# duyhominhnguyen/conan-fgw

Hardware: AMD Instinct MI355X
Metric: molecules/s (K=5 conformers) (higher is better)
Workload: dtype f32

## Files before the change

### conan-fgw_amd/csrc/fgw.hip

```cpp
#include "fgw_coupling.h"
#ifdef CONAN_FGW_PROFILE
FGW_PROF_ACCESSOR(conan_debug_fgw_prof_large)
FGW_PROF_TRACE_ACCESSOR(conan_debug_fgw_trace_large)
#endif

namespace {

__global__ void k_fgw_init(const float *__restrict__ Cs, const float *__restrict__ init_C, const float *__restrict__ init_Y,
                           FgwDims D, int max_iter, double *__restrict__ Cw, double *__restrict__ Yw, int *__restrict__ active,
                           int *__restrict__ info, float *__restrict__ errs, float *__restrict__ Yout, float *__restrict__ Cout, FgwAdj adj) {
    const int b = blockIdx.x;
    const int NN = D.N * D.N, Nd = D.N * D.d;
    if (!init_C && adj.rowptr) {
        const int N = D.N, g = b * D.K;
        for (int t = threadIdx.x; t < NN; t += blockDim.x) Cout[(size_t)b * NN + t] = 0.f;
        __syncthreads();
        const int lo = adj.gptr[g], n = min(adj.gptr[g + 1] - lo, N);
        for (int e = adj.rowptr[lo] + (int)threadIdx.x; e < adj.rowptr[lo + n]; e += blockDim.x) {
            const int i = adj.tgt[e] - lo, j = adj.col[e] - lo;
            if (i >= 0 && i < N && j >= 0 && j < N) atomicAdd(&Cout[(size_t)b * NN + j * N + i], 1.0f);
        }
        __threadfence_block();
        __syncthreads();
        for (int t = threadIdx.x; t < NN; t += blockDim.x) Cw[(size_t)b * NN + t] = (double)Cout[(size_t)b * NN + t];
// ... 587 lines not shown
    w.redo = region(BK * 4 + 512);
    w.dense = region(ragged ? al256(BK * NN * sizeof(float)) : 0);
    w.asym = region(solver == 2 && symmetric != 1 ? al256(conan_fgw_bapg_asym_scratch_bytes(B, K, N)) : 0);
    w.total = end;
    return w;
}

enum class FgwPath {
    Small,
    Big,
    General,
    Bapg
};
struct FgwPlan {
    FgwPath path;
    int mode;
    size_t lds_bytes;
    bool kl, ppa, asym;
    bool y_from_t;
    size_t big_bytes;
    bool big_u8, big_wpc2, big_ordered;
};

template <int M>
void launch_general(const FgwCall &c, const FgwPlan &pl, int outer, int y_zero, const int *only) {
    auto go = [&](auto kernel, int blocks) {
        launch_lds(kernel, blocks, 64 * GEN_NW, pl.lds_bytes, c.s, c.Ys, c.Cs, c.ps, c.p, c.D, c.prm, outer, y_zero | (c.symmetric < 0 ? 2 : 0), c.Cw,
                   c.Yw, c.active, c.T, c.info, c.scratch, c.Ypart, c.Cpart, only, c.adj);
    };
    if (only) go(k_fgw_coupling<M, false, GEN_NW, true>, (c.D.B * c.D.K + 63) / 64);
    else with_flags([&](auto KL, auto PPA, auto ASYM) { go(k_fgw_coupling<M, KL.value, GEN_NW, false, PPA.value, ASYM.value>, c.D.B * c.D.K); },
                    pl.kl, pl.ppa, pl.asym);
}

int fgw_fwd_impl(const float *Ys, const float *Cs, const float *ps, const float *p, const float *lambdas, const float *init_C,
                 const float *init_Y, int B, int K, int N, int d, const conan_fgw_params *params, float *Y, float *C, float *T, float *T_iter,
                 int *info, float *errs, void *workspace, void *stream, FgwAdj adj, int solver, int symmetric) {
    if (solver < 0 || solver > 2 || symmetric < -1 || symmetric > 1) return CONAN_E_BADARG;
    if (!Ys || !(Cs || (adj.gptr && adj.rowptr && adj.col && adj.tgt)) || !params || !Y || !C || !T || !info || !errs || !workspace || B <= 0 || K <= 0 || N <= 0 || d <= 0)
        return CONAN_E_BADARG;
    if (params->max_iter <= 0 || params->num_iter_max <= 0) return CONAN_E_BADARG;
    if (params->fixed_features && !init_Y) return CONAN_E_BADARG;
    if (params->loss_fun != 0 && params->loss_fun != 1) return CONAN_E_BADARG;
    const bool ragged = adj.rowptr != nullptr, small = conan_fgw_small_supported(N, d), kl = params->loss_fun != 0;
    const bool model = solver == 0 && symmetric == 1;
    const FgwWorkspace w = fgw_workspace(B, K, N, d, ragged, solver, symmetric);
    const size_t NN = (size_t)N * N, NP = (size_t)N * pitch_of(N);
    FgwCall c{};
    c.Ys = Ys; c.Cs = Cs; c.ps = ps; c.p = p; c.lambdas = lambdas; c.init_C = init_C; c.init_Y = init_Y;
    c.D = FgwDims{B, K, N, d, pitch_of(N)};
    c.prm = *params;
    c.adj = adj;
    c.symmetric = symmetric;
    c.Y = Y; c.C = C; c.T = T; c.info = info; c.errs = errs;
    c.Cw = ws_at<double>(workspace, w.Cw); c.Yw = ws_at<double>(workspace, w.Yw); c.active = ws_at<int>(workspace, w.active);
    c.scratch = ws_at<char>(workspace, w.scratch); c.scratch_stride = coupling_scratch_stride(NP);
    c.Ypart = ws_at<fgw_part_t>(workspace, w.Ypart); c.Cpart = ws_at<fgw_part_t>(workspace, w.Cpart);
    c.redo = ws_at<int>(workspace, w.redo);
    c.asym_scratch = ws_at<char>(workspace, w.asym);
    c.s = as_stream(stream);
    if (ragged) {
        c.prm.cs_small_int = 1;
        c.adj.dense = ws_at<float>(workspace, w.dense);
        if (!(model && !kl && (small ? conan_fgw_fast_supported(N, d, 1) : big_lds(N, true) <= LDS_LIMIT))) {
            k_adj_dense<<<B * K, 256, 0, c.s>>>(c.adj, N);
            c.Cs = c.adj.dense;
            c.adj.rowptr = nullptr;
        }
    }
    if (!model) c.adj = FgwAdj{};
    if (c.adj.rowptr && !kl && (B & 7) == 0 && B <= 4096 && (small || (CONAN_FGW_BIG_ORDER && big_lds(N, true) <= LDS_LIMIT)))
        c.adj.order = ws_at<int>(workspace, w.order);

    FgwPlan pl{};
    pl.kl = kl; pl.ppa = solver == 1; pl.asym = symmetric != 1;
    pl.big_u8 = c.prm.cs_small_int != 0;
    pl.big_bytes = big_lds(N, pl.big_u8);
    pl.path = solver == 2 ? FgwPath::Bapg : model && small ? FgwPath::Small : model && !kl && pl.big_bytes <= LDS_LIMIT ? FgwPath::Big : FgwPath::General;
    pl.mode = general_mode(N, &pl.lds_bytes);
    pl.big_wpc2 = BIG_WPC2 && (B * K <= CONAN_FGW_WPC2_MAX || (CONAN_FGW_WPC2_ORDERED && c.adj.order));
    pl.big_ordered = c.adj.order != nullptr && (B * K & 7) == 0 && pl.big_wpc2 && pl.big_u8;
    pl.y_from_t = pl.path == FgwPath::Small && !c.prm.fixed_features && conan_fgw_update_chunk(K, N, d, B) > 0;
    if (pl.path == FgwPath::Small) { c.zvec = ws_at<double>(workspace, w.zvec); c.yvec = ws_at<double>(workspace, w.yvec); }

    if (pl.path == FgwPath::Small) conan_fgw_small_prepare(c);
    else k_fgw_init<<<B, 256, 0, c.s>>>(c.Cs, init_C, init_Y, c.D, c.prm.max_iter, c.Cw, c.Yw, c.active, info, errs, Y, C, c.adj);
    const FastConst fc = fast_const(c.prm, N);
    for (int outer = 0; outer < c.prm.max_iter; ++outer) {
        const int y_zero = (outer == 0 && !init_Y) ? 1 : 0;
        const int *only = nullptr;
        if (pl.path == FgwPath::Big) {
            auto big = [&](auto kernel) {
                launch_lds(kernel, B * K, 64 * GEN_NW, pl.big_bytes, c.s, c.Ys, c.Cs, c.ps, c.p, c.D, c.prm, fc, outer, y_zero, c.Cw, c.Yw, c.active, c.T,
                           c.info, c.scratch, c.Ypart, c.Cpart, c.redo, c.adj);
            };
            if (pl.big_ordered) big(k_fgw_coupling_big<GEN_NW, true, 2, true>);
            else if (pl.big_u8) { if (pl.big_wpc2) big(k_fgw_coupling_big<GEN_NW, true, 2, false>); else big(k_fgw_coupling_big<GEN_NW, true, 3, false>); }
            else { if (pl.big_wpc2) big(k_fgw_coupling_big<GEN_NW, false, 2, false>); else big(k_fgw_coupling_big<GEN_NW, false, 3, false>); }
            only = c.redo;
        }
        if (pl.path == FgwPath::Small) conan_fgw_small_coupling(c, outer, y_zero, pl.y_from_t ? nullptr : c.Ypart);
        else if (pl.path == FgwPath::Bapg) conan_fgw_bapg_coupling(c, outer, y_zero);
        else if (pl.mode == 2) launch_general<2>(c, pl, outer, y_zero, only);
        else if (pl.mode == 1) launch_general<1>(c, pl, outer, y_zero, only);
        else launch_general<0>(c, pl, outer, y_zero, only);
        if (T_iter)
            (void)hipMemcpyAsync(T_iter + (size_t)outer * B * K * NN, T, (size_t)B * K * NN * sizeof(float), hipMemcpyDeviceToDevice, c.s);
        conan_fgw_small_update(c, outer, pl.y_from_t);
    }
    CONAN_LAUNCH_CHECK();
    return CONAN_OK;
}

}

extern "C" {

long long conan_fgw_workspace_bytes(int B, int K, int N, int d, int ragged, int solver, int symmetric) {
    if (ragged != 0 && ragged != 1) return 0;
    return (long long)fgw_workspace(B, K, N, d, ragged != 0, solver, symmetric).total;
}

int conan_fgw_barycenter_fwd(const float *Ys, const float *Cs, const float *ps, const float *p, const float *lambdas,
                             const float *init_C, const float *init_Y, int B, int K, int N, int d,
                             const conan_fgw_params *params, int solver, int symmetric, float *Y, float *C, float *T, float *T_iter,
                             int *info, float *errs, void *workspace, void *stream) {
    return fgw_fwd_impl(Ys, Cs, ps, p, lambdas, init_C, init_Y, B, K, N, d, params, Y, C, T, T_iter, info, errs, workspace, stream, FgwAdj{}, solver,
                        symmetric);
}

int conan_fgw_barycenter_fwd_ragged(const float *Ys, const int *graph_ptr, const int *rowptr, const int *col, const int *tgt, const float *ps,
                                    const float *p, const float *lambdas, const float *init_C, const float *init_Y, int B, int K, int N, int d,
                                    const conan_fgw_params *params, int solver, int symmetric, float *Y, float *C, float *T, float *T_iter,
                                    int *info, float *errs, void *workspace, void *stream) {
    return fgw_fwd_impl(Ys, nullptr, ps, p, lambdas, init_C, init_Y, B, K, N, d, params, Y, C, T, T_iter, info, errs, workspace, stream,
                        FgwAdj{graph_ptr, rowptr, col, tgt, nullptr, nullptr}, solver, symmetric);
}

int conan_fgw_barycenter_bwd(const float *T, const float *dY, const float *p, const float *lambdas, int B, int K,
                             int N, int d, float *dYs, void *stream) {
    if (!T || !dY || !dYs || B <= 0 || K <= 0 || N <= 0 || d <= 0) return CONAN_E_BADARG;
    const size_t bw_lds = ((size_t)N * N + (size_t)N * d) * sizeof(float);
    if (bw_lds <= 64 * 1024) k_fgw_bwd<true><<<B * K, 256, bw_lds, as_stream(stream)>>>(T, dY, p, lambdas, K, N, d, dYs);
    else k_fgw_bwd<false><<<B * K, 256, 0, as_stream(stream)>>>(T, dY, p, lambdas, K, N, d, dYs);
    CONAN_LAUNCH_CHECK();
    return CONAN_OK;
}

int conan_fgw_densify(const float *feat, const int *graph_ptr, const int *rowptr, const int *col, int num_graphs,
                      int N, int d, float shift, float a, float b, float *Ys, float *Cs, float *minmax, void *stream) {
    if (!feat || !graph_ptr || !Ys || !minmax || num_graphs <= 0 || N <= 0 || d <= 0 || (Cs && (!rowptr || !col))) return CONAN_E_BADARG;
    k_densify<<<num_graphs, 256, 0, as_stream(stream)>>>(feat, graph_ptr, rowptr, col, N, d, shift, a, b, Ys, Cs, minmax);
    CONAN_LAUNCH_CHECK();
    return CONAN_OK;
}

int conan_fgw_densify_bwd(const float *feat, const float *dYs, const int *graph_ptr, const float *minmax,
                          int num_graphs, int N, int d, float shift, float a, float b, float *dfeat, void *stream) {
    if (!feat || !dYs || !graph_ptr || !minmax || !dfeat || num_graphs <= 0 || N <= 0 || d <= 0) return CONAN_E_BADARG;
    k_densify_bwd<<<num_graphs, 256, 0, as_stream(stream)>>>(feat, dYs, graph_ptr, minmax, N, d, shift, a, b, dfeat);
    CONAN_LAUNCH_CHECK();
    return CONAN_OK;
}

int conan_fgw_readout_fwd(const float *Y, int B, int K, int N, int d, int mode, float *out, void *stream) {
    if (!Y || !out || B <= 0 || K <= 0 || N <= 0 || d <= 0 || mode < 0 || mode > 1) return CONAN_E_BADARG;
// ... 15 lines not shown
```

### conan-fgw_amd/csrc/fgw_common.h

```cpp
#pragma once
#include <type_traits>
#include "common.h"

#ifdef CONAN_FGW_PROFILE
static __device__ long long g_fgw_prof[32];
#define FGW_PROF_ACCESSOR(name)                                                          \
    extern "C" int name(long long *out, int reset) {                                     \
        if (out && hipMemcpyFromSymbol(out, HIP_SYMBOL(g_fgw_prof), sizeof(long long) * 32) != hipSuccess) return -2; \
        if (reset) { long long z[32] = {0}; if (hipMemcpyToSymbol(HIP_SYMBOL(g_fgw_prof), z, sizeof(z)) != hipSuccess) return -2; } \
        return 0;                                                                        \
    }
static __device__ long long g_fgw_trace[2 + 6 * 8192];
#define FGW_PROF_TRACE_ACCESSOR(name)                                                    \
    extern "C" int name(long long *out, int reset) {                                     \
        if (out && hipMemcpyFromSymbol(out, HIP_SYMBOL(g_fgw_trace), sizeof(long long) * (2 + 6 * 8192)) != hipSuccess) return -2; \
        if (reset) { long long z[2] = {0, 0}; if (hipMemcpyToSymbol(HIP_SYMBOL(g_fgw_trace), z, sizeof(z)) != hipSuccess) return -2; } \
        return 0;                                                                        \
    }
#define FGW_PROF_TRACE(tag)                                                              \
    do {                                                                                 \
        if (threadIdx.x == 0) {                                                          \
            const unsigned long long i_ = atomicAdd(reinterpret_cast<unsigned long long *>(&g_fgw_trace[0]), 1ull); \
            if (i_ < 8192) {                                                             \
                long long *r_ = &g_fgw_trace[2 + 6 * i_];                                \
                r_[0] = (long long)blockIdx.x; r_[1] = (long long)(tag);                 \
                r_[2] = (long long)__builtin_amdgcn_s_getreg(4 | (31 << 11));            \
                r_[3] = (long long)__builtin_amdgcn_s_getreg(20 | (31 << 11));           \
                r_[4] = prof_w0; r_[5] = wall_clock64();                                 \
            }                                                                            \
        }                                                                                \
    } while (0)
#define FGW_PROF_DECL long long prof_t = wall_clock64(); const long long prof_w0 = prof_t, prof_c0 = clock64(); long long prof_acc[11] = {0, 0, 0, 0, 0, 0, 0, 0, 0, 0, 0}
#define FGW_PROF(k)                                                                      \
    do {                                                                                 \
        const long long t_ = wall_clock64();                                             \
        prof_acc[k] += t_ - prof_t;                                                      \
        prof_t = t_;                                                                     \
    } while (0)
#define FGW_PROF_FLUSH                                                                   \
    do {                                                                                 \
        if (threadIdx.x == 0) {                                                          \
            for (int k_ = 0; k_ < 11; ++k_) atomicAdd(reinterpret_cast<unsigned long long *>(&g_fgw_prof[k_]), (unsigned long long)prof_acc[k_]); \
            atomicAdd(reinterpret_cast<unsigned long long *>(&g_fgw_prof[20]), (unsigned long long)(clock64() - prof_c0));      \
            atomicAdd(reinterpret_cast<unsigned long long *>(&g_fgw_prof[21]), (unsigned long long)(wall_clock64() - prof_w0)); \
        }                                                                                \
    } while (0)
#elif defined(CONAN_FGW_MARK)
#define FGW_PROF_DECL
#define FGW_PROF(k) asm volatile("; FGWMARK " #k)
#define FGW_PROF_FLUSH
#define FGW_PROF_TRACE(tag)
#else
#define FGW_PROF_DECL
#define FGW_PROF(k)
#define FGW_PROF_FLUSH
#define FGW_PROF_TRACE(tag)
#endif

constexpr int FGW_THREADS = 256;
constexpr int FGW_WAVES = FGW_THREADS / 64;

typedef double fgw_part_t;

__host__ __device__ inline int fgw_pitch(int N) { return N | 1; }
struct FgwDims {
    int B, K, N, d, P;
};

struct FgwPair {
    const float *M;
    float *errs;
    int nerr;
};

__device__ __forceinline__ bool fgw_active(const int *__restrict__ active, int B, int b, int outer) {
    const int *a = active + ((outer + 1) & 1) * 2 * B;
    return (a[b] | a[B + b]) != 0;
}
__device__ __forceinline__ void fgw_active_init(int *__restrict__ active, int B, int b) { active[2 * B + b] = 1; active[3 * B + b] = 1; }

struct FgwAdj {
    const int *gptr, *rowptr, *col, *tgt;
    float *dense;
    int *order;
};
template <int NT>
__device__ __forceinline__ void adj_scatter_lds_bytes(const FgwAdj &A, int g, int N, int P, unsigned char *m, int tid) {
    const int lo = A.gptr[g], n = min(A.gptr[g + 1] - lo, N);
    const int e0 = A.rowptr[lo], e1 = A.rowptr[lo + n];
    for (int e = e0 + tid; e < e1; e += NT) {
        const int i = A.tgt[e] - lo, j = A.col[e] - lo;
        if (i >= 0 && i < N && j >= 0 && j < N) {
            const unsigned o = (unsigned)(j * P + i);
            atomicAdd(reinterpret_cast<unsigned *>(m + (o & ~3u)), 1u << (8 * (o & 3u)));
        }
    }
}
template <int NT>
__device__ __forceinline__ const float *adj_dense_slice(const FgwAdj &A, int g, int N, int tid) {
    float *dst = A.dense + (size_t)g * N * N;
    for (int t = tid; t < N * N; t += NT) dst[t] = 0.f;
    __syncthreads();
    const int lo = A.gptr[g], n = min(A.gptr[g + 1] - lo, N);
    const int e0 = A.rowptr[lo], e1 = A.rowptr[lo + n];
    for (int e = e0 + tid; e < e1; e += NT) {
        const int i = A.tgt[e] - lo, j = A.col[e] - lo;
        if (i >= 0 && i < N && j >= 0 && j < N) atomicAdd(&dst[j * N + i], 1.0f);
    }
    __threadfence_block();
    __syncthreads();
    return dst;
}

struct FastConst {
    double two_alpha, one_m_alpha, four_alpha_inv_eps, inv_eps, inner_tol, stop_thr, inv_n;
};
inline FastConst fast_const(const conan_fgw_params &prm, int N) {
    const double alpha = (double)prm.alpha, inv_eps = 1.0 / (double)prm.epsilon;
    return FastConst{2.0 * alpha, 1.0 - alpha, 4.0 * alpha * inv_eps, inv_eps, (double)prm.inner_tol, (double)prm.stop_thr, 1.0 / (double)N};
}

__device__ __forceinline__ double exp_acc(double x) {
    if (x < -745.0) return 0.0;
    const double t = x * 1.4426950408889634074;
    const double n = rint(t);
    const float f = (float)(t - n);
    const float e = __builtin_amdgcn_exp2f(f);
    return ldexp((double)e, (int)n);
}

__device__ __forceinline__ double exp_fast(double x) {
    const double xc = fmin(fmax(x, -700.0), 700.0);
    const double t = xc * 1.4426950408889634074;
    const double sh = t + 6755399441055744.0;
    const int n = __double2loint(sh);
    const double f = t - (sh - 6755399441055744.0);
    const double e = (double)__builtin_amdgcn_exp2f((float)f);
    const double scale = __hiloint2double((n + 1023) << 20, 0);
    const double r = e * scale;
    return x > -700.0 ? (x < 700.0 ? r : __builtin_inf()) : 0.0;
}

__device__ __forceinline__ double rcp_pos(double s) {
    double r = __builtin_amdgcn_rcp(s);
    r = fma(fma(-s, r, 1.0), r, r);
    r = fma(fma(-s, r, 1.0), r, r);
    return r;
}

__device__ __forceinline__ double log_acc(double s) {
    const double y0 = (double)(__builtin_amdgcn_logf((float)s) * 0.693147180559945309f);
    const double r = s * exp_acc(-y0) - 1.0;
    return y0 + (r - 0.5 * r * r);
}

__device__ __forceinline__ double wave_sum_d(double v) {
#pragma unroll
    for (int o = 32; o > 0; o >>= 1) v += __shfl_xor(v, o, 64);
    return v;
}
__device__ __forceinline__ double wave_max_d(double v) {
#pragma unroll
    for (int o = 32; o > 0; o >>= 1) { double w = __shfl_xor(v, o, 64); v = w > v ? w : v; }
    return v;
}

template <int NW = FGW_WAVES>
__device__ __forceinline__ double block_sum_d(double v, double *red) {
// ... 842 lines not shown
```

### conan-fgw_amd/csrc/fgw_small.hip

```cpp
#include "fgw_common.h"

#ifdef CONAN_FGW_PROFILE
FGW_PROF_ACCESSOR(conan_debug_fgw_prof)
FGW_PROF_TRACE_ACCESSOR(conan_debug_fgw_trace)
#endif

namespace {

constexpr int SK_SCRATCH_DOUBLES = 3 * 256 + 2 * 64;

template <int R, bool KL, bool SECOND = false>
__global__ void __launch_bounds__(FGW_THREADS, (SECOND || R > 9) ? 1 : 3) k_fgw_coupling_small(
    const float *__restrict__ Ys, const float *__restrict__ Cs, const float *__restrict__ ps, const float *__restrict__ pb,
    FgwDims D, conan_fgw_params prm, int outer, int y_zero, const double *__restrict__ Cw, const double *__restrict__ Yw,
    const int *__restrict__ active, float *__restrict__ Tw, int *__restrict__ info, fgw_part_t *__restrict__ Ypart,
    fgw_part_t *__restrict__ Cpart, const double *__restrict__ zvec, const double *__restrict__ yvec, const int *__restrict__ only, FgwAdj adj) {
    extern __shared__ __attribute__((aligned(16))) char smem[];
    auto solve = [&](const int cid) {
    const int b = cid / D.K, s = cid % D.K;
    if (!fgw_active(active, D.B, b, outer)) return;
    const int N = D.N, P = D.P, d = D.d;
    const int NN = N * N, NP = N * P;
    const int tid = threadIdx.x, lane = tid & 63, w = __builtin_amdgcn_readfirstlane(tid >> 6);
    const bool lane_ok = lane < N;
// ... 276 lines not shown

    if (!prm.fixed_features && Ypart) {
        fgw_part_t *Yp = Ypart + ((size_t)b * D.K + s) * N * d;
        if (z_lds) {
            const int Nd = N * d;
            for (int t0 = tid; t0 < Nd; t0 += 4 * FGW_THREADS) {
                float zv[4];
#pragma unroll
                for (int u = 0; u < 4; ++u) { const int t = t0 + u * FGW_THREADS; zv[u] = Z[t < Nd ? t : Nd - 1]; }
#pragma unroll
                for (int u = 0; u < 4; ++u) { const int t = t0 + u * FGW_THREADS; if (t < Nd) Zl2[t] = zv[u]; }
            }
            __syncthreads();
            mm_lds<FGW_WAVES, false>(N, d, N, Tl, P, Zl2, d, [&](int i, int c, double v) { Yp[(size_t)i * d + c] = (fgw_part_t)v; }, border_prepare(N, d));
        } else {
            mm_f64(N, d, N, [&](int i, int k) { return (double)Tl[i * P + k]; }, [&](int k, int c) { return (double)Z[(size_t)k * d + c]; },
                   [&](int i, int c, double v) { Yp[(size_t)i * d + c] = (fgw_part_t)v; });
        }
    }
    FGW_PROF(9);
    if (!prm.fixed_structure) {
        fgw_part_t *Cp = Cpart + ((size_t)b * D.K + s) * NN;
        if constexpr (KL)
            mm_f64(N, N, N, [&](int i, int k) { return (double)Tl[i * P + k]; },
                   [&](int k, int j) { const double cv = (double)C2l[k * P + j]; return log(cv > 1e-15 ? cv : 1e-15); },
                   [&](int i, int j, double v) { Al[i * P + j] = v; }, bnn);
        else
            mm_lds<FGW_WAVES, false>(N, N, N, Tl, P, C2l, P, [&](int i, int j, double v) { Al[i * P + j] = v; }, bnn);
        __syncthreads();
        mm_lds<FGW_WAVES, true>(N, N, N, Al, P, Tl, P, [&](int i, int j, double v) { Cp[i * N + j] = (fgw_part_t)v; }, bnn);
    }
    FGW_PROF(10);
    FGW_PROF_FLUSH;
    };
    if constexpr (!SECOND) solve(blockIdx.x);
    else {
        const int total = D.B * D.K, base = (int)blockIdx.x * 64, l = (int)threadIdx.x & 63;
        unsigned long long m = __ballot(base + l < total && only[base + l < total ? base + l : 0] != 0);
        while (m) {
            const int k = __ffsll((long long)m) - 1;
            m &= m - 1;
            solve(base + k);
            __syncthreads();
        }
    }
}

template <int R> struct FastCfg {
    static constexpr int OCC = R <= 9 ? 5 : (R <= 12 ? 2 : 1);
};
inline int fast_tiles_per_wave(int N) {
    const int Mc = (N >> 4) << 4;
    const bool border = (N - Mc) * N + Mc * (N - Mc) <= FGW_WAVES * 32 && Mc > 0;
    const int q = border ? N >> 4 : (N + 15) >> 4;
    return (q * q + FGW_WAVES - 1) / FGW_WAVES;
}
constexpr int FAST_VEC_DOUBLES = 128 + 256;
constexpr int FAST_SK_DOUBLES = 2 * 256 + 2 * 64;

struct FastLds {
    int npa;
    size_t off_t, off_c2, off_red, off_vec, off_sk, off_rs, bytes;
    bool vec_alias, sk_alias;
};
template <typename C2T>
__host__ __device__ inline FastLds fast_lds(int N) {
    FastLds L;
    const int NP = N * fgw_pitch(N);
    L.npa = (NP + 1) & ~1;
    size_t o = (size_t)3 * L.npa * 8;
    L.off_t = o; o += ((size_t)NP * 4 + 15) & ~(size_t)15;
    L.off_c2 = o; o += ((size_t)NP * sizeof(C2T) + 15) & ~(size_t)15;
    L.off_red = o; o += 64;
    L.vec_alias = (size_t)NP * 4 >= FAST_VEC_DOUBLES * 8;
    L.sk_alias = L.npa >= FAST_SK_DOUBLES;
    L.off_vec = L.vec_alias ? L.off_t : o; if (!L.vec_alias) o += FAST_VEC_DOUBLES * 8;
    L.off_sk = L.sk_alias ? (size_t)L.npa * 8 : o; if (!L.sk_alias) o += FAST_SK_DOUBLES * 8;
    const bool rs_alias = (size_t)NP * sizeof(C2T) >= (size_t)4 * N * 8;
    L.off_rs = rs_alias ? L.off_c2 : o; if (!rs_alias) o += (size_t)4 * N * 8;
    L.bytes = o;
    return L;
}

template <int R, int MAXT, typename C2T>
__global__ void __launch_bounds__(FGW_THREADS, FastCfg<R>::OCC) k_fgw_coupling_fast(
    const float *__restrict__ Ys, const float *__restrict__ Cs, const float *__restrict__ ps, const float *__restrict__ pb,
    FgwDims D, conan_fgw_params prm, FastConst fc, int outer, int y_zero, const double *__restrict__ Cw, const double *__restrict__ Yw,
    const int *__restrict__ active, float *__restrict__ Tw, int *__restrict__ info, fgw_part_t *__restrict__ Ypart,
    fgw_part_t *__restrict__ Cpart, const double *__restrict__ zvec, const double *__restrict__ yvec, int *__restrict__ redo, FgwAdj adj) {
    extern __shared__ __attribute__((aligned(16))) char smem[];
    int cid = (gridDim.x & 7) == 0 ? xcd_contiguous_block((int)blockIdx.x, (int)gridDim.x) : (int)blockIdx.x;
    if (adj.order && (gridDim.x & 7) == 0) {
        const int x = (int)blockIdx.x & 7, pblk = (int)blockIdx.x >> 3;
        cid = adj.order[x + 8 * (pblk / D.K)] * D.K + pblk % D.K;
    }
    const int b = cid / D.K, s = cid % D.K;
    if (!fgw_active(active, D.B, b, outer)) return;
    const int N = D.N, P = D.P, d = D.d;
    const int NN = N * N;
    const int tid = threadIdx.x, lane = tid & 63, w = __builtin_amdgcn_readfirstlane(tid >> 6);
    FGW_PROF_DECL;

    const FastLds L = fast_lds<C2T>(N);
    double *C1l = reinterpret_cast<double *>(smem);
    double *AKl = C1l + L.npa;
    double *Bl = AKl + L.npa;
    float *Tl = reinterpret_cast<float *>(smem + L.off_t);
    C2T *C2l = reinterpret_cast<C2T *>(smem + L.off_c2);
    double *red = reinterpret_cast<double *>(smem + L.off_red);
    float *t_dummy = reinterpret_cast<float *>(red + 7);
    double *pq = reinterpret_cast<double *>(smem + L.off_vec);
    double *vec4 = pq + 128;
    double *bufC = reinterpret_cast<double *>(smem + L.off_sk);
    double *bufR = bufC + 256;
    double *fvP = bufR + 256;
    double *gvP = fvP + 64;
    double *Yl = AKl;
    float *Zl = reinterpret_cast<float *>(C1l);
    const bool yz_lds = d <= 2 * P;

    const float *Z = Ys + ((size_t)b * D.K + s) * N * d;
    const float *C2 = Cs + ((size_t)b * D.K + s) * NN;
    const double *C1 = Cw + (size_t)b * NN;
    const double *Y = Yw + (size_t)b * N * d;
    float *Tg = Tw + ((size_t)b * D.K + s) * NN;

    constexpr int EPT = (16 * R * R + FGW_THREADS - 1) / FGW_THREADS;
    const int e_dq = FGW_THREADS / N, e_dr = FGW_THREADS - e_dq * N;
    const int e_i0 = tid / N, e_j0 = tid - e_i0 * N;
    auto for_entries = [&](auto fn) {
        int i = e_i0, j = e_j0;
#pragma unroll
        for (int u = 0; u < EPT; ++u) {
            if (tid + u * FGW_THREADS < NN) fn(u, i * P + j);
            j += e_dr; i += e_dq;
            if (j >= N) { j -= N; ++i; }
        }
    };
    const bool warm = outer > 0 && prm.warmstart;
    const bool stage_yz = d <= 2 * P && !y_zero;
    const bool ragged = sizeof(C2T) == 1 && adj.rowptr != nullptr;
    float c2v[EPT];
#pragma unroll
    for (int u = 0; u < EPT; ++u) { const int t = tid + u * FGW_THREADS; c2v[u] = ragged ? 0.f : C2[t < NN ? t : NN - 1]; }
    double c1v[EPT];
    float tv[EPT];
    auto load_c1_t = [&]() {
#pragma unroll
        for (int u = 0; u < EPT; ++u) {
            const int t = tid + u * FGW_THREADS, tc = t < NN ? t : NN - 1;
            c1v[u] = C1[tc]; tv[u] = warm ? Tg[tc] : 0.f;
        }
    };
    if (!stage_yz) load_c1_t();
    const double p_own = tid < N ? (pb ? (double)pb[(size_t)b * N + tid] : fc.inv_n) : 1.0;
    const double q_own = tid < N ? (ps ? (double)ps[((size_t)b * D.K + s) * N + tid] : fc.inv_n) : 1.0;
    double vec_own;
    {
        const int v = tid >> 6, i = tid & 63;
        const double *src = (v == 0 || v == 2) ? yvec + (size_t)b * 2 * N + (v == 0 ? N : 0) : zvec + ((size_t)b * D.K + s) * 2 * N + (v == 1 ? N : 0);
        vec_own = src[i < N ? i : N - 1];
        vec_own = i < N ? vec_own : 0.0;
    }
    int nb = N;
    if (ragged) nb = min(adj.gptr[cid + 1] - adj.gptr[cid], N);
    const bool pad_try = !pb && !ps && !Ypart && !prm.fixed_structure && !prm.fixed_features;
    auto c1_block_ok = [&](int nb_) {
        auto near = [](double a, double b_) { return fabs(a - b_) <= 1e-9 * (fabs(b_) + 1e-30) || a == b_; };
        bool ok = true;
        const int lc = lane < N ? lane : N - 1;
        const double c_nb = C1[(size_t)nb_ * N + lc];
        const double cbb = __shfl(c_nb, nb_, 64);
        const double want = lane < nb_ ? c_nb : cbb;
        for (int r = nb_ + 1 + w; r < N; r += FGW_WAVES) ok = ok && (lane >= N || near(C1[(size_t)r * N + lc], want));
        ok = ok && (lane < nb_ || lane >= N || near(c_nb, cbb));
        const int mcol = N - nb_;
        for (int k = w; k < nb_; k += FGW_WAVES) {
            const double v = C1[(size_t)k * N + nb_ + (lane < mcol ? lane : 0)];
            ok = ok && near(v, __shfl(v, 0, 64));
        }
        return ok;
    };
    bool pad_ok = pad_try && ragged && N - nb >= 2 && nb >= 1;
    if (pad_ok) pad_ok = c1_block_ok(nb);
    if (stage_yz) {
        const int Nd = N * d;
        for (int t0 = tid; t0 < Nd; t0 += 4 * FGW_THREADS) {
            double yv[4]; float zv[4];
#pragma unroll
            for (int u = 0; u < 4; ++u) { const int t = t0 + u * FGW_THREADS, tc = t < Nd ? t : Nd - 1; yv[u] = Y[tc]; zv[u] = Z[tc]; }
#pragma unroll
            for (int u = 0; u < 4; ++u) { const int t = t0 + u * FGW_THREADS; if (t < Nd) { Yl[t] = yv[u]; Zl[t] = zv[u]; } }
        }
    }
    if (tid < 64) { pq[tid] = p_own; pq[64 + tid] = q_own; }
    vec4[tid] = vec_own;
    for_entries([&](int u, int o) { C2l[o] = (C2T)c2v[u]; if (!stage_yz) C1l[o] = c1v[u]; });
    if constexpr (sizeof(C2T) == 1) {
        if (ragged) {
            __syncthreads();
            adj_scatter_lds_bytes<FGW_THREADS>(adj, cid, N, P, reinterpret_cast<unsigned char *>(C2l), tid);
        }
    }
    __syncthreads();
    int n_real;
    {
        const bool nz = lane < N && C2l[lane] != (C2T)0;
        n_real = 1 + __popcll(__ballot(nz));
    }
    bool complete;
    {
        bool ok = true;
        int i = e_i0, j = e_j0;
#pragma unroll
        for (int u = 0; u < EPT; ++u) {
            if (tid + u * FGW_THREADS < NN) ok = ok && (C2l[i * P + j] == (C2T)((i != j && i < n_real && j < n_real) ? 1 : 0));
            j += e_dr; i += e_dq;
            if (j >= N) { j -= N; ++i; }
        }
        complete = __syncthreads_and(ok) != 0 && n_real >= 2;
    }
    double *rsum = reinterpret_cast<double *>(smem + L.off_rs);
    if (!ragged) {
        int mx = 1;
        int i = e_i0, j = e_j0;
#pragma unroll
        for (int u = 0; u < EPT; ++u) {
            if (tid + u * FGW_THREADS < NN && C2l[i * P + j] != (C2T)0) mx = max(mx, max(i, j) + 1);
            j += e_dr; i += e_dq;
            if (j >= N) { j -= N; ++i; }
        }
#pragma unroll
        for (int o = 32; o > 0; o >>= 1) mx = max(mx, __shfl_xor(mx, o, 64));
        int *ired = reinterpret_cast<int *>(red);
        if (lane == 0) ired[w] = mx;
        __syncthreads();
        nb = max(max(ired[0], ired[1]), max(ired[2], ired[3]));
        __syncthreads();
        pad_ok = pad_try && N - nb >= 2 && nb >= 1;
        if (pad_ok) pad_ok = c1_block_ok(nb);
    }
    int m_pad = 0;
    if (pad_try && N - nb >= 2 && nb >= 1) {
        auto nearf = [](double a, double b_) { return fabs(a - b_) <= 1e-9 * (fabs(b_) + 1e-30) || a == b_; };
        bool ok = pad_ok;
        for (int r = nb + 1 + w; r < N; r += FGW_WAVES)
            for (int c = lane; c < d; c += 64) {
                if (stage_yz) {
                    ok = ok && nearf((double)Zl[r * d + c], (double)Zl[nb * d + c]) && nearf(Yl[r * d + c], Yl[nb * d + c]);
                } else {
                    ok = ok && nearf((double)Z[(size_t)r * d + c], (double)Z[(size_t)nb * d + c]);
                    if (!y_zero) ok = ok && nearf(Y[(size_t)r * d + c], Y[(size_t)nb * d + c]);
                }
            }
        if (__syncthreads_and(ok) != 0) m_pad = N - nb;
    }
    const int Nx = m_pad ? nb + 1 : N;
    const double mult = m_pad ? (double)m_pad : 1.0;
    FGW_PROF(0);
    const double qj = pq[64 + lane] * ((m_pad && lane == nb) ? mult : 1.0);
    const double pi_l = pq[lane] * ((m_pad && lane == nb) ? mult : 1.0);
    const double *r1v = vec4, *r2v = vec4 + 64, *y2v = vec4 + 128, *z2v = vec4 + 192;
    auto base_of = [&](int i, int j, double dot) {
        double m = -2.0 * dot; m += y2v[i]; m += z2v[j];
        m = m > 0.0 ? m : 0.0;
        return fc.two_alpha * (r1v[i] + r2v[j]) + fc.one_m_alpha * m;
    };
    if (y_zero) {
        int i = e_i0, j = e_j0;
#pragma unroll
        for (int u = 0; u < EPT; ++u) {
            if (tid + u * FGW_THREADS < NN) Bl[i * P + j] = base_of(i, j, 0.0);
            j += e_dr; i += e_dq;
            if (j >= N) { j -= N; ++i; }
        }
    } else if (stage_yz) {
        mm_lds2<FGW_WAVES, MAXT, 0, true, true>(Nx, Nx, d, Yl, d, Zl, d, [&]() { load_c1_t(); __syncthreads(); },
                                                [&](int i, int j, double v) { Bl[i * P + j] = base_of(i, j, v); });
        for_entries([&](int u, int o) { C1l[o] = c1v[u]; });
    } else {
        mm_f64(Nx, Nx, d, [&](int i, int k) { return Y[(size_t)i * d + k]; }, [&](int k, int j) { return (double)Z[(size_t)j * d + k]; },
               [&](int i, int j, double v) { Bl[i * P + j] = base_of(i, j, v); });
    }
    __syncthreads();
    FGW_PROF(1);
    if (warm) {
        if (m_pad) {
            int i = e_i0, j = e_j0;
#pragma unroll
            for (int u = 0; u < EPT; ++u) {
                if (tid + u * FGW_THREADS < NN) Tl[i * P + j] = (float)((double)tv[u] * ((i == nb ? mult : 1.0) * (j == nb ? mult : 1.0)));
                j += e_dr; i += e_dq;
                if (j >= N) { j -= N; ++i; }
            }
// ... 196 lines not shown
    }
    FGW_PROF(9);
    if (!prm.fixed_structure) {
        fgw_part_t *Cp = Cpart + ((size_t)b * D.K + s) * NN;
        if (complete) {
            {
                const int lc = lane < Nx ? lane : Nx - 1;
                const float *tr = Tl + lc * P + w;
                double p0 = 0.0, p1 = 0.0;
#pragma unroll
                for (int r = 0; r < R; ++r) {
                    const int q = w + 4 * r;
                    if (q < n_real) { if (r & 1) p1 += (double)tr[4 * r]; else p0 += (double)tr[4 * r]; }
                }
                if (lane < Nx) rsum[w * N + lane] = p0 + p1;
            }
            __syncthreads();
            mm_lds2<FGW_WAVES, 1, 0, true, false>(Nx, Nx, n_real, Tl, P, Tl, P, [] {}, [&](int i, int j, double v) {
                const double ti = ((rsum[i] + rsum[N + i]) + rsum[2 * N + i]) + rsum[3 * N + i];
                const double tj = ((rsum[j] + rsum[N + j]) + rsum[2 * N + j]) + rsum[3 * N + j];
                if (m_pad) Bl[i * P + j] = ti * tj - v;
                else Cp[i * N + j] = (fgw_part_t)(ti * tj - v);
            });
        } else {
            mm_lds2<FGW_WAVES, 1, 0, false, false>(Nx, Nx, Nx, Tl, P, C2l, P, [] {}, [&](int i, int j, double v) { AKl[i * P + j] = v; });
            __syncthreads();
            mm_lds2<FGW_WAVES, 1, 0, true, false>(Nx, Nx, Nx, AKl, P, Tl, P, [] {}, [&](int i, int j, double v) {
                if (m_pad) Bl[i * P + j] = v;
                else Cp[i * N + j] = (fgw_part_t)v;
            });
        }
        if (m_pad) {
            __syncthreads();
            const double im = 1.0 / mult;
            int i = tid / N, j = tid - i * N;
            const int dq = FGW_THREADS / N, dr = FGW_THREADS - dq * N;
            for (int t = tid; t < NN; t += FGW_THREADS) {
                Cp[t] = (fgw_part_t)(Bl[min(i, nb) * P + min(j, nb)] * ((i >= nb ? im : 1.0) * (j >= nb ? im : 1.0)));
                j += dr; i += dq;
                if (j >= N) { j -= N; ++i; }
            }
        }
    }
    FGW_PROF(10);
    FGW_PROF_FLUSH;
    FGW_PROF_TRACE(Nx | (cpt << 8) | (sk_total << 20));
}

template <int NT>
__device__ __forceinline__ void molecule_vectors(const double *__restrict__ Y, const double *__restrict__ C, const float *__restrict__ p, int N,
                                                 int d, bool kl, double *__restrict__ out, int which = 2) {
    constexpr int LPI = NT / 64;
    const int i = (int)threadIdx.x / LPI, sub = (int)threadIdx.x % LPI;
    double y2 = 0.0, r1 = 0.0;
    if (i < N) {
        if (which != 1)
            for (int c = sub; c < d; c += LPI) { const double v = Y[(size_t)i * d + c]; y2 += v * v; }
        if (which != 0)
            for (int k = sub; k < N; k += LPI) {
                const double c1 = C[i * N + k], pk = p ? (double)p[k] : 1.0 / (double)N;
                r1 += (kl ? c1 * log(c1 + 1e-15) - c1 : c1 * c1) * pk;
            }
    }
#pragma unroll
    for (int o = 1; o < LPI; o <<= 1) { y2 += __shfl_xor(y2, o, 64); r1 += __shfl_xor(r1, o, 64); }
    if (i < N && sub == 0) { if (which != 1) out[i] = y2; if (which != 0) out[N + i] = r1; }
}

__global__ void __launch_bounds__(256) k_fgw_small_vectors(const float *__restrict__ Ys, const float *__restrict__ Cs, const float *__restrict__ ps,
                                                           const float *__restrict__ pb, FgwDims D, int kl, double *__restrict__ Cw,
                                                           double *__restrict__ Yw, double *__restrict__ zvec, double *__restrict__ yvec,
                                                           const float *__restrict__ init_C, const float *__restrict__ init_Y, int max_iter,
                                                           int *__restrict__ active, int *__restrict__ info, float *__restrict__ errs,
                                                           float *__restrict__ Yout, float *__restrict__ Cout, FgwAdj adj) {
    const int b = blockIdx.x / D.K, s = blockIdx.x % D.K;
    const int N = D.N, d = D.d;
    __shared__ __attribute__((aligned(16))) unsigned char cm[64 * 65 + 16];
    const int Pm = D.P;
    if (adj.rowptr) {
        for (int t = threadIdx.x; t < (64 * 65 + 16) / 4; t += 256) reinterpret_cast<unsigned *>(cm)[t] = 0u;
        __syncthreads();
        adj_scatter_lds_bytes<256>(adj, (int)blockIdx.x, N, Pm, cm, (int)threadIdx.x);
        __syncthreads();
    }
    if (s == 0) {
        const int NN = N * N, Nd = N * d;
        const float *c0 = init_C ? init_C + (size_t)b * NN : Cs + (size_t)b * D.K * NN;
        for (int t = threadIdx.x; t < NN; t += 256) {
            const float cv = (!init_C && adj.rowptr) ? (float)cm[(t / N) * Pm + (t % N)] : c0[t];
            Cw[(size_t)b * NN + t] = (double)cv; Cout[(size_t)b * NN + t] = cv;
        }
        for (int t = threadIdx.x; t < Nd; t += 256) {
            const float y = init_Y ? init_Y[(size_t)b * Nd + t] : 0.f;
            Yw[(size_t)b * Nd + t] = (double)y; Yout[(size_t)b * Nd + t] = y;
        }
        if (threadIdx.x == 0) { fgw_active_init(active, D.B, b); info[b * 4 + 0] = 0; info[b * 4 + 1] = 0; info[b * 4 + 2] = 0; info[b * 4 + 3] = 0; }
        for (int t = threadIdx.x; t < 2 * max_iter; t += 256) errs[(size_t)b * 2 * max_iter + t] = __builtin_nanf("");
        __syncthreads();
    }
    const float *Z = Ys + ((size_t)b * D.K + s) * N * d;
    const float *C2 = Cs + ((size_t)b * D.K + s) * N * N;
    const float *q = ps ? ps + ((size_t)b * D.K + s) * N : nullptr;
    const int j = (int)threadIdx.x >> 2, sub = (int)threadIdx.x & 3;
    double z2 = 0.0, r2 = 0.0;
    if (j < N) {
        for (int c = sub; c < d; c += 4) { const double v = (double)Z[(size_t)j * d + c]; z2 += v * v; }
        for (int k = sub; k < N; k += 4) {
            const double c2 = adj.rowptr ? (double)cm[j * Pm + k] : (double)C2[j * N + k], qk = q ? (double)q[k] : 1.0 / (double)N;
            r2 += qk * (kl ? c2 : c2 * c2);
        }
    }
    z2 += __shfl_xor(z2, 1, 64); z2 += __shfl_xor(z2, 2, 64);
    r2 += __shfl_xor(r2, 1, 64); r2 += __shfl_xor(r2, 2, 64);
    double *zo = zvec + ((size_t)b * D.K + s) * 2 * N;
    if (j < N && sub == 0) { zo[j] = z2; zo[N + j] = r2; }
    if (s == 0)
        molecule_vectors<256>(Yw + (size_t)b * N * d, Cw + (size_t)b * N * N, pb ? pb + (size_t)b * N : nullptr, N, d, kl != 0, yvec + (size_t)b * 2 * N);
    if (adj.order && blockIdx.x == gridDim.x - 1) fgw_order_by_size<256>(adj, D.B, D.K, (int)threadIdx.x);
}

constexpr int UPD_THREADS = 512;
template <bool Y_FROM_T>
__global__ void __launch_bounds__(UPD_THREADS) k_fgw_update_parts(
    const float *__restrict__ pb, const float *__restrict__ lambdas, FgwDims D, conan_fgw_params prm, int outer,
    const fgw_part_t *__restrict__ Ypart, const fgw_part_t *__restrict__ Cpart, double *__restrict__ Cw, double *__restrict__ Yw,
    int *__restrict__ active, int *__restrict__ info, float *__restrict__ errs, float *__restrict__ Yout, float *__restrict__ Cout,
    double *__restrict__ yvec, const float *__restrict__ Tw, const float *__restrict__ Ys, int chunk) {
    __shared__ double red[UPD_THREADS / 64 + 1];
    extern __shared__ __attribute__((aligned(16))) char usmem[];
    const int part = (int)blockIdx.x >= D.B ? 1 : 0;
    const int b = (int)blockIdx.x - part * D.B;
    const int N = D.N, d = D.d, K = D.K, NN = N * N, Nd = N * d;
    const int tid = threadIdx.x;
    int *flag_out = active + (outer & 1) * 2 * D.B + part * D.B + b;
    if (!fgw_active(active, D.B, b, outer)) {
        if (tid == 0) *flag_out = 0;
        return;
    }
    constexpr int U = 4;
    double e2 = 0.0;
    if (part == 0) {
        if (!prm.fixed_features) {
            double *Yb = Yw + (size_t)b * Nd;
            if constexpr (Y_FROM_T) {
                float *Tl = reinterpret_cast<float *>(usmem), *Zl = Tl + (size_t)chunk * NN;
                const int lane = tid & 63, wave = __builtin_amdgcn_readfirstlane(tid >> 6), li = lane & 15, lk = lane >> 4;
                const int Mq = (N + 15) >> 4, Nq = (d + 15) >> 4;
                constexpr int NWU = UPD_THREADS / 64, TW = 2;
                for (int t0 = 0; t0 < Mq * Nq; t0 += NWU * TW) {
                    int ti0[TW], tj0[TW], tic[TW], tjc[TW];
                    bool mine[TW];
                    f64x4 sum[TW];
#pragma unroll
                    for (int w = 0; w < TW; ++w) {
                        const int t = t0 + wave + w * NWU;
                        mine[w] = t < Mq * Nq;
                        ti0[w] = mine[w] ? (t / Nq) << 4 : 0; tj0[w] = mine[w] ? (t % Nq) << 4 : 0;
                        tic[w] = min(ti0[w] + li, N - 1); tjc[w] = min(tj0[w] + li, d - 1);
                        sum[w] = f64x4{0.0, 0.0, 0.0, 0.0};
                    }
                    for (int s0 = 0; s0 < K; s0 += chunk) {
                        const int cs = min(chunk, K - s0);
                        __syncthreads();
                        const float *tg = Tw + ((size_t)b * K + s0) * NN, *zg = Ys + ((size_t)b * K + s0) * Nd;
                        auto stage = [&](const float *__restrict__ src, float *dst, int n) {
                            constexpr int SB = 12;
// ... 55 lines not shown
                        }
                    }
#pragma unroll
                    for (int u = 0; u < U; ++u) {
                        const int t = t0 + u * UPD_THREADS;
                        if (t < Nd) {
                            const double df = acc[u] - old[u];
                            e2 += df * df;
                            Yb[t] = acc[u];
                            Yout[(size_t)b * Nd + t] = (float)acc[u];
                        }
                    }
                }
            }
        }
    } else if (!prm.fixed_structure) {
        double *Cb = Cw + (size_t)b * NN;
        for (int t0 = tid; t0 < NN; t0 += U * UPD_THREADS) {
            double acc[U], old[U];
#pragma unroll
            for (int u = 0; u < U; ++u) {
                const int t = t0 + u * UPD_THREADS;
                acc[u] = 0.0; old[u] = 0.0;
                if (t < NN) {
                    old[u] = Cb[t];
                    for (int s = 0; s < K; ++s) {
                        const double lam = lambdas ? (double)lambdas[s] : 1.0 / (double)K;
                        acc[u] += lam * Cpart[((size_t)b * K + s) * NN + t];
                    }
                }
            }
#pragma unroll
            for (int u = 0; u < U; ++u) {
                const int t = t0 + u * UPD_THREADS;
                if (t < NN) {
                    const int i = t / N, j = t - i * N;
                    const double pi = pb ? (double)pb[(size_t)b * N + i] : 1.0 / (double)N;
                    const double pj = pb ? (double)pb[(size_t)b * N + j] : 1.0 / (double)N;
                    const double cn = pi * pj > 0.0 ? (prm.loss_fun ? exp(acc[u] / (pi * pj)) : acc[u] / (pi * pj)) : 0.0;
                    const double df = cn - old[u];
                    e2 += df * df;
                    Cb[t] = cn;
                    Cout[(size_t)b * NN + t] = (float)cn;
                }
            }
        }
    }
    const double err = sqrt(block_sum_d<UPD_THREADS / 64>(e2, red));
    if (yvec) molecule_vectors<UPD_THREADS>(Yw + (size_t)b * Nd, Cw + (size_t)b * NN, pb ? pb + (size_t)b * N : nullptr, N, d, prm.loss_fun != 0,
                                            yvec + (size_t)b * 2 * N, part);
    if (tid == 0) {
        errs[((size_t)b * 2 + part) * prm.max_iter + outer] = (float)err;
        info[b * 4 + 0] = outer + 1;
        *flag_out = err > (double)prm.tol ? 1 : 0;
    }
}

inline size_t small_lds(int N, int d) {
    const size_t NP = (size_t)N * fgw_pitch(N);
    (void)d; return NP * 8 * 4 + (256 + 128 + 8 + (NP >= (size_t)SK_SCRATCH_DOUBLES ? 0 : SK_SCRATCH_DOUBLES)) * 8 + NP * 4 * 2;
}

}

bool conan_fgw_small_supported(int N, int d) { return N <= 64 && small_lds(N, d) <= 160 * 1024; }

void conan_fgw_small_prepare(const FgwCall &c) {
    k_fgw_small_vectors<<<c.D.B * c.D.K, 256, 0, c.s>>>(c.Ys, c.Cs, c.ps, c.p, c.D, c.prm.loss_fun, c.Cw, c.Yw, c.zvec, c.yvec, c.init_C, c.init_Y,
                                                       c.prm.max_iter, c.active, c.info, c.errs, c.Y, c.C, c.adj);
}

template <class F>
static void with_rows(int R, F &&f) {
    if (R <= 6) f(std::integral_constant<int, 6>{});
    else if (R <= 9) f(std::integral_constant<int, 9>{});
    else if (R <= 12) f(std::integral_constant<int, 12>{});
    else f(std::integral_constant<int, 16>{});
}

template <int R, typename C2T>
static void launch_fast(const FgwCall &c, int outer, int y_zero, fgw_part_t *Ypart) {
    const FgwDims &D = c.D;
    const int tpw = fast_tiles_per_wave(D.N);
    auto go = [&](auto kernel) {
        launch_lds(kernel, D.B * D.K, FGW_THREADS, fast_lds<C2T>(D.N).bytes, c.s, c.Ys, c.Cs, c.ps, c.p, D, c.prm, fast_const(c.prm, D.N), outer,
                   y_zero, c.Cw, c.Yw, c.active, c.T, c.info, Ypart, c.Cpart, c.zvec, c.yvec, c.redo, c.adj);
    };
    if constexpr (R <= 6) go(k_fgw_coupling_fast<R, 1, C2T>);
    else if constexpr (R <= 12) { if (tpw <= 1) go(k_fgw_coupling_fast<R, 1, C2T>); else go(k_fgw_coupling_fast<R, 3, C2T>); }
    else { if (tpw <= 1) go(k_fgw_coupling_fast<R, 1, C2T>); else if (tpw <= 3) go(k_fgw_coupling_fast<R, 3, C2T>); else go(k_fgw_coupling_fast<R, 4, C2T>); }
}

bool conan_fgw_fast_supported(int N, int d, int small_int) {
    if (N > 64 || N < 4) return false;
    const size_t lds = small_int ? fast_lds<unsigned char>(N).bytes : fast_lds<float>(N).bytes;
    return lds <= 160 * 1024 && d >= 1;
}

void conan_fgw_small_coupling(const FgwCall &c, int outer, int y_zero, fgw_part_t *Ypart) {
    const FgwDims &D = c.D;
    const size_t lds = small_lds(D.N, D.d);
    const int grid = D.B * D.K;
    const bool kl = c.prm.loss_fun != 0;
    with_rows((D.N + 3) / 4, [&](auto R) {
        const int *only = nullptr;
        if (!kl && conan_fgw_fast_supported(D.N, D.d, c.prm.cs_small_int)) {
            if (c.prm.cs_small_int) launch_fast<R.value, unsigned char>(c, outer, y_zero, Ypart);
            else launch_fast<R.value, float>(c, outer, y_zero, Ypart);
            only = c.redo;
        }
        auto exact = [&](auto kernel, int blocks) {
            launch_lds(kernel, blocks, FGW_THREADS, lds, c.s, c.Ys, c.Cs, c.ps, c.p, D, c.prm, outer, y_zero, c.Cw, c.Yw, c.active, c.T, c.info, Ypart,
                       c.Cpart, c.zvec, c.yvec, only, c.adj);
        };
        if (kl) exact(k_fgw_coupling_small<R.value, true, false>, grid);
        else if (only) exact(k_fgw_coupling_small<R.value, false, true>, (grid + 63) / 64);
        else exact(k_fgw_coupling_small<R.value, false, false>, grid);
    });
}

void conan_fgw_small_update(const FgwCall &c, int outer, bool y_from_t) {
    const FgwDims &D = c.D;
    const int chunk = y_from_t ? conan_fgw_update_chunk(D.K, D.N, D.d, D.B) : 0;
    if (chunk > 0)
        launch_lds(k_fgw_update_parts<true>, 2 * D.B, UPD_THREADS, (size_t)chunk * ((size_t)D.N * D.N + (size_t)D.N * D.d) * 4, c.s, c.p, c.lambdas, D,
                   c.prm, outer, nullptr, c.Cpart, c.Cw, c.Yw, c.active, c.info, c.errs, c.Y, c.C, c.yvec, c.T, c.Ys, chunk);
    else
        k_fgw_update_parts<false><<<2 * D.B, UPD_THREADS, 0, c.s>>>(c.p, c.lambdas, D, c.prm, outer, c.Ypart, c.Cpart, c.Cw, c.Yw, c.active, c.info, c.errs,
                                                                     c.Y, c.C, c.yvec, nullptr, nullptr, 0);
}

int conan_fgw_update_chunk(int K, int N, int d, int B) {
    if (N > 64) return 0;
    const size_t per = ((size_t)N * N + (size_t)N * d) * 4, budget = (2 * B <= 256 ? 144 : 72) * 1024;
    if (per > budget) return 0;
    const int c = (int)(budget / per);
    return c < K ? c : K;
}
```

Baseline: 118,200.

## Precompute per-graph adjacency facts once and reuse them in fast coupling kernel

The prepare kernel now computes each graph's real node count and a 'complete graph' flag from the scattered byte adjacency. For non-complete graphs it also stores the byte image in scratch. The fast coupling kernel, run every outer iteration, reads these facts and copies the cached image instead of re-scattering the CSR adjacency and recomputing n_real/completeness. This removes atomics and a reduction per iteration, at the cost of scratch traffic and more template instantiations. It relies on the scratch region not being overwritten between prepare and coupling.

```diff
diff --git a/conan-fgw_amd/csrc/fgw.hip b/conan-fgw_amd/csrc/fgw.hip
--- a/conan-fgw_amd/csrc/fgw.hip
+++ b/conan-fgw_amd/csrc/fgw.hip
@@ -693,6 +693,7 @@
     pl.big_ordered = c.adj.order != nullptr && (B * K & 7) == 0 && pl.big_wpc2 && pl.big_u8;
     pl.y_from_t = pl.path == FgwPath::Small && !c.prm.fixed_features && conan_fgw_update_chunk(K, N, d, B) > 0;
     if (pl.path == FgwPath::Small) { c.zvec = ws_at<double>(workspace, w.zvec); c.yvec = ws_at<double>(workspace, w.yvec); }
+    if (CONAN_FGW_GRAPH_FACTS && pl.path == FgwPath::Small && c.adj.rowptr) c.adj.facts = c.scratch;
 
     if (pl.path == FgwPath::Small) conan_fgw_small_prepare(c);
     else k_fgw_init<<<B, 256, 0, c.s>>>(c.Cs, init_C, init_Y, c.D, c.prm.max_iter, c.Cw, c.Yw, c.active, info, errs, Y, C, c.adj);
diff --git a/conan-fgw_amd/csrc/fgw_common.h b/conan-fgw_amd/csrc/fgw_common.h
--- a/conan-fgw_amd/csrc/fgw_common.h
+++ b/conan-fgw_amd/csrc/fgw_common.h
@@ -83,7 +83,24 @@
     const int *gptr, *rowptr, *col, *tgt;
     float *dense;
     int *order;
+    char *facts;
 };
+#ifndef CONAN_FGW_GRAPH_FACTS
+#define CONAN_FGW_GRAPH_FACTS 1
+#endif
+constexpr int FGW_FACTS_IMAGE_OFFSET = 16;
+template <int NT>
+__device__ __forceinline__ int fgw_graph_facts_word(const unsigned char *m, int N, int P, int tid) {
+    const int lane = tid & 63;
+    const int n_real = 1 + __popcll(__ballot(lane < N && m[lane] != 0));
+    bool ok = true;
+    for (int t = tid; t < N * N; t += NT) {
+        const int i = t / N, j = t - i * N;
+        ok = ok && (m[i * P + j] == (unsigned char)((i != j && i < n_real && j < n_real) ? 1 : 0));
+    }
+    const bool complete = __syncthreads_and(ok) != 0 && n_real >= 2;
+    return (n_real & 0xff) | (complete ? 0x100 : 0);
+}
 template <int NT>
 __device__ __forceinline__ void adj_scatter_lds_bytes(const FgwAdj &A, int g, int N, int P, unsigned char *m, int tid) {
     const int lo = A.gptr[g], n = min(A.gptr[g + 1] - lo, N);
diff --git a/conan-fgw_amd/csrc/fgw_small.hip b/conan-fgw_amd/csrc/fgw_small.hip
--- a/conan-fgw_amd/csrc/fgw_small.hip
+++ b/conan-fgw_amd/csrc/fgw_small.hip
@@ -382,7 +382,7 @@
     return L;
 }
 
-template <int R, int MAXT, typename C2T>
+template <int R, int MAXT, typename C2T, bool FACTS = false>
 __global__ void __launch_bounds__(FGW_THREADS, FastCfg<R>::OCC) k_fgw_coupling_fast(
     const float *__restrict__ Ys, const float *__restrict__ Cs, const float *__restrict__ ps, const float *__restrict__ pb,
     FgwDims D, conan_fgw_params prm, FastConst fc, int outer, int y_zero, const double *__restrict__ Cw, const double *__restrict__ Yw,
@@ -439,10 +439,13 @@
     };
     const bool warm = outer > 0 && prm.warmstart;
     const bool stage_yz = d <= 2 * P && !y_zero;
-    const bool ragged = sizeof(C2T) == 1 && adj.rowptr != nullptr;
+    static_assert(!FACTS || sizeof(C2T) == 1, "graph facts describe the byte image");
+    const bool ragged = FACTS || (sizeof(C2T) == 1 && adj.rowptr != nullptr);
     float c2v[EPT];
-#pragma unroll
-    for (int u = 0; u < EPT; ++u) { const int t = tid + u * FGW_THREADS; c2v[u] = ragged ? 0.f : C2[t < NN ? t : NN - 1]; }
+    if constexpr (!FACTS) {
+#pragma unroll
+        for (int u = 0; u < EPT; ++u) { const int t = tid + u * FGW_THREADS; c2v[u] = ragged ? 0.f : C2[t < NN ? t : NN - 1]; }
+    }
     double c1v[EPT];
     float tv[EPT];
     auto load_c1_t = [&]() {
@@ -463,7 +466,23 @@
         vec_own = i < N ? vec_own : 0.0;
     }
     int nb = N;
-    if (ragged) nb = min(adj.gptr[cid + 1] - adj.gptr[cid], N);
+    constexpr int IMW = ((4 * R * (4 * R + 1) + 3) / 4 + FGW_THREADS - 1) / FGW_THREADS;
+    constexpr bool facts = FACTS;
+    int fword = 0;
+    if constexpr (facts) {
+        const char *fp = adj.facts + (size_t)cid * coupling_scratch_stride((size_t)N * P);
+        const int2 fv = *reinterpret_cast<const int2 *>(fp);
+        nb = __builtin_amdgcn_readfirstlane(fv.x); fword = __builtin_amdgcn_readfirstlane(fv.y);
+        const int nw = (N * P + 3) / 4;
+        if (!(fword & 0x100)) {
+#pragma unroll
+            for (int u = 0; u < IMW; ++u) {
+                const int t = tid + u * FGW_THREADS;
+                if (t < nw) reinterpret_cast<unsigned *>(C2l)[t] = reinterpret_cast<const unsigned *>(fp + FGW_FACTS_IMAGE_OFFSET)[t];
+            }
+        }
+    } else if (ragged) nb = min(adj.gptr[cid + 1] - adj.gptr[cid], N);
+    (void)fword;
     const bool pad_try = !pb && !ps && !Ypart && !prm.fixed_structure && !prm.fixed_features;
     auto c1_block_ok = [&](int nb_) {
         auto near = [](double a, double b_) { return fabs(a - b_) <= 1e-9 * (fabs(b_) + 1e-30) || a == b_; };
@@ -495,21 +514,19 @@
     }
     if (tid < 64) { pq[tid] = p_own; pq[64 + tid] = q_own; }
     vec4[tid] = vec_own;
-    for_entries([&](int u, int o) { C2l[o] = (C2T)c2v[u]; if (!stage_yz) C1l[o] = c1v[u]; });
-    if constexpr (sizeof(C2T) == 1) {
+    for_entries([&](int u, int o) { if constexpr (!facts) C2l[o] = (C2T)c2v[u]; if (!stage_yz) C1l[o] = c1v[u]; });
+    if constexpr (sizeof(C2T) == 1 && !facts) {
         if (ragged) {
             __syncthreads();
             adj_scatter_lds_bytes<FGW_THREADS>(adj, cid, N, P, reinterpret_cast<unsigned char *>(C2l), tid);
         }
     }
     __syncthreads();
-    int n_real;
-    {
+    int n_real = fword & 0xff;
+    bool complete = (fword & 0x100) != 0;
+    if constexpr (!facts) {
         const bool nz = lane < N && C2l[lane] != (C2T)0;
         n_real = 1 + __popcll(__ballot(nz));
-    }
-    bool complete;
-    {
         bool ok = true;
         int i = e_i0, j = e_j0;
 #pragma unroll
@@ -872,6 +889,17 @@
         __syncthreads();
         adj_scatter_lds_bytes<256>(adj, (int)blockIdx.x, N, Pm, cm, (int)threadIdx.x);
         __syncthreads();
+        if (adj.facts) {
+            char *fp = adj.facts + (size_t)blockIdx.x * coupling_scratch_stride((size_t)N * Pm);
+            const int word = fgw_graph_facts_word<256>(cm, N, Pm, (int)threadIdx.x);
+            if (threadIdx.x == 0) {
+                reinterpret_cast<int *>(fp)[0] = min(adj.gptr[blockIdx.x + 1] - adj.gptr[blockIdx.x], N);
+                reinterpret_cast<int *>(fp)[1] = word;
+            }
+            if (!(word & 0x100))
+                for (int t = threadIdx.x; t < (N * Pm + 3) / 4; t += 256)
+                    reinterpret_cast<unsigned *>(fp + FGW_FACTS_IMAGE_OFFSET)[t] = reinterpret_cast<const unsigned *>(cm)[t];
+        }
     }
     if (s == 0) {
         const int NN = N * N, Nd = N * d;
@@ -1093,13 +1121,21 @@
 static void launch_fast(const FgwCall &c, int outer, int y_zero, fgw_part_t *Ypart) {
     const FgwDims &D = c.D;
     const int tpw = fast_tiles_per_wave(D.N);
+    constexpr bool U8 = sizeof(C2T) == 1;
+    const bool facts = U8 && c.adj.facts != nullptr;
     auto go = [&](auto kernel) {
         launch_lds(kernel, D.B * D.K, FGW_THREADS, fast_lds<C2T>(D.N).bytes, c.s, c.Ys, c.Cs, c.ps, c.p, D, c.prm, fast_const(c.prm, D.N), outer,
                    y_zero, c.Cw, c.Yw, c.active, c.T, c.info, Ypart, c.Cpart, c.zvec, c.yvec, c.redo, c.adj);
     };
-    if constexpr (R <= 6) go(k_fgw_coupling_fast<R, 1, C2T>);
-    else if constexpr (R <= 12) { if (tpw <= 1) go(k_fgw_coupling_fast<R, 1, C2T>); else go(k_fgw_coupling_fast<R, 3, C2T>); }
-    else { if (tpw <= 1) go(k_fgw_coupling_fast<R, 1, C2T>); else if (tpw <= 3) go(k_fgw_coupling_fast<R, 3, C2T>); else go(k_fgw_coupling_fast<R, 4, C2T>); }
+    auto pick = [&](auto F) {
+        constexpr bool FA = decltype(F)::value;
+        if constexpr (R <= 6) go(k_fgw_coupling_fast<R, 1, C2T, FA>);
+        else if constexpr (R <= 12) { if (tpw <= 1) go(k_fgw_coupling_fast<R, 1, C2T, FA>); else go(k_fgw_coupling_fast<R, 3, C2T, FA && R != 9>); }
+        else { if (tpw <= 1) go(k_fgw_coupling_fast<R, 1, C2T, FA>); else if (tpw <= 3) go(k_fgw_coupling_fast<R, 3, C2T, FA>); else go(k_fgw_coupling_fast<R, 4, C2T, FA>); }
+    };
+    if constexpr (U8 && CONAN_FGW_GRAPH_FACTS != 0) { if (facts) { pick(std::true_type{}); return; } }
+    (void)facts;
+    pick(std::false_type{});
 }
 
 bool conan_fgw_fast_supported(int N, int d, int small_int) {
```

Result: no change. 119,300 (median of 6 runs) (+0.9%).
